# lmcinnes/enstop

Measured on AMD Instinct MI355X. Metric: EM iterations/sec, higher is better.
Workload: dtype f32; 1 GPU; 1M x 100k, 100M nnz; corpus=independent Zipf tokens (SURVEY 8d), nnz=100435863, k=64, schedule=fused, parallelism=single fit

## Files before the change

### enstop_amd/_lib.py

```python
import ctypes as C
import os

import numpy as np

_HERE = os.path.dirname(os.path.abspath(__file__))
LIB_PATH = os.environ.get("ENSTOP_AMD_LIB", os.path.join(_HERE, "libplsa_hip.so"))

PLSA_FUSED = 1
PLSA_TRACE_LL = 4
PLSA_SW_LL_ONLY = 8
PLSA_STOP_NO_ZERO_ARM = 16
PLSA_SHARDED = 64
PLSA_REFERENCE_SUMS = 256
PLSA_REFERENCE_LL = 512

_i32p = np.ctypeslib.ndpointer(np.int32, flags="C_CONTIGUOUS")
_i64p = np.ctypeslib.ndpointer(np.int64, flags="C_CONTIGUOUS")
_f32p = np.ctypeslib.ndpointer(np.float32, flags="C_CONTIGUOUS")
_f64p = np.ctypeslib.ndpointer(np.float64, flags="C_CONTIGUOUS")
_ctx = C.c_void_p
_i64 = C.c_int64
_i32 = C.c_int32
_vp = C.c_void_p

# ... 40 lines not shown
    "plsa_comm_init": (C.c_int, [_ctx, C.c_char_p, _i32, _i32]),
    "plsa_comm_destroy": (C.c_int, [_ctx]),
    "plsa_comm_info": (C.c_int, [_ctx, C.POINTER(_i32), C.POINTER(_i32)]),
    "plsa_comm_barrier": (C.c_int, [_ctx]),
    "plsa_stack_reserve": (C.c_int, [_ctx, C.c_int64, C.c_int64, C.c_int32, C.POINTER(C.c_void_p)]),
    "plsa_comm_allgather_stack": (C.c_int, [_ctx, C.c_int64, C.c_int64, C.c_int32, C.POINTER(C.POINTER(C.c_float))]),
    "plsa_comm_allgather_stack_to": (C.c_int, [_ctx, _i64, _i64, _i32, _f32p]),
    "plsa_comm_allgather_host": (C.c_int, [_ctx, _vp, _i64, _vp]),
    "plsa_comm_allreduce_f64": (C.c_int, [_ctx, _f64p, _i64, _i32]),
    "plsa_comm_broadcast_host": (C.c_int, [_ctx, _vp, _i64, _i32]),
    "plsa_allreduce_accumulator": (C.c_int, [_ctx]),
    "plsa_reference_chain_info": (C.c_int, [_ctx, C.POINTER(_i64), C.POINTER(_i64), C.POINTER(_i32)]),
    "plsa_placement_info": (C.c_int, [_ctx, C.POINTER(_i32), C.POINTER(C.c_double), C.POINTER(C.c_double)]),
    "plsa_schedule_info": (C.c_int, [_ctx, C.POINTER(_i32), C.POINTER(C.c_double), C.POINTER(_i32), C.POINTER(_i32),
                                     C.POINTER(C.c_int64)]),
    "plsa_release_scratch": (C.c_int, [_ctx]),
    "plsa_timing_enable": (C.c_int, [_ctx, _i32]),
    "plsa_timing_reset": (C.c_int, [_ctx]),
    "plsa_timing_get": (C.c_int, [_ctx, C.c_char_p, C.POINTER(C.c_double), C.POINTER(_i64)]),
    "plsa_timing_report": (C.c_int, [_ctx, C.c_char_p, _i64]),
    "plsa_measure_stream_bandwidth": (C.c_int, [_ctx, _i64, _i32, _i32, C.POINTER(C.c_double)]),
    "plsa_all_pairs_hellinger": (C.c_int, [_ctx, C.c_void_p, _i64, _i64, _f64p]),
    "plsa_all_pairs_kl": (C.c_int, [_ctx, C.c_void_p, _i64, _i64, _f64p]),
    "plsa_cluster_representatives": (C.c_int, [_ctx, C.c_void_p, _i64, _i64, _i32p, _vp, _i32, _f32p]),
    "plsa_host_normalize_rows": (None, [_f64p, _i64, _i64]),
    "plsa_host_mt19937_jump": (C.c_int, [C.POINTER(C.c_uint32), _i32]),
    "plsa_generate_synthetic": (C.c_int, [_ctx, _i64, _i64, _i64, C.c_double, C.c_uint64,
                                          C.POINTER(_i64)]),
    "plsa_generate_synthetic_topics": (C.c_int, [_ctx, _i64, _i64, _i64, C.c_double, C.c_uint64, _i32, C.c_double,
                                                 C.c_double, C.POINTER(_i64)]),
# ... 54 lines not shown
```

### enstop_amd/csrc/plsa_hip.hip

```cpp
#include <hip/hip_runtime.h>
#include <hipcub/hipcub.hpp>
#include <rccl/rccl.h>

#include <algorithm>
#include <cmath>
#include <cstdarg>
#include <cstdio>
#include <cstdlib>
#include <cstring>
#include <mutex>
#include <string>
#include <thread>
#include <type_traits>
#include <vector>

#include "../../include/plsa_hip.h"
#include "../../include/plsa_hip_diag.h"
#include "mt_jump.hpp"
#include "plsa_kernels.hpp"
#include "plsa_ref_kernels.hpp"
#include "plsa_synth.hpp"

using plsa::i64;

// ... 30 lines not shown

    i64 bn = 0, bm = 0, bnnz = 0;
    DevBuf b_indptr, b_col, b_val;
    bool active_is_base = true;
    i64 n = 0, m = 0, nnz = 0;
    DevBuf a_indptr, a_col, a_val, rowidx;
    const int *indptr = nullptr, *col = nullptr;
    const float *val = nullptr;
    bool rowidx_valid = false;

    bool csc_valid = false;
    int seg = 256, seg_override = 0, struct_lpn = 0;
    i64 n_items = 0;
    DevBuf colptr, csc_row, csc_val, csc_pos, item_first, item_col, item_start, item_order, partial, heavy_cols;
    bool use_item_order = true, xcd_split = true;
    int chunks_per_lane = 2;
    int row_lpn = 1, row_ch = 1;
    bool row_shape_8x2 = true;
    bool p_borrowed = false;
    bool p_lent = false;
    int e_rows = -1;
    int mt_streams = 256;
    i64 mt_min_blocks = 4096;
    int heavy_items = 32, n_heavy = 0;

    bool force_wide = false;
    bool ritems_valid = false, use_ritems = false;
    int rseg = 64, rseg_override = 0, ritems_mode = -1;
    i64 n_ritems = 0;
    DevBuf ritem_first, ritem_row, ritem_start, rpartial;
// ... 384 lines not shown
int grid_for(plsa_ctx *c, i64 work_items, int items_per_block) {
    i64 need = (work_items + items_per_block - 1) / items_per_block;
    if (need < 1) need = 1;
    return (int)std::min<i64>(need, c->grid_cap);
}

void set_active_pointers(plsa_ctx *c) {
    if (c->active_is_base) {
        c->indptr = c->b_indptr.as<int>(); c->col = c->b_col.as<int>(); c->val = c->b_val.as<float>();
        c->n = c->bn; c->m = c->bm; c->nnz = c->bnnz;
    } else {
        c->indptr = c->a_indptr.as<int>(); c->col = c->a_col.as<int>(); c->val = c->a_val.as<float>();
    }
    c->rowidx_valid = false;
    c->csc_valid = false;
    c->roworder_valid = false;
    c->ritems_valid = false;
    c->eitems_valid = false;
    c->p_valid = false;
    c->ref_pairs_off = false;
    c->ref_heavy_valid = false;
    c->ref_tsum_valid = false;
}

int ensure_rowidx(plsa_ctx *c) {
    if (c->rowidx_valid) return 0;
    CHK(ensure(c, c->rowidx, sizeof(int) * (size_t)c->nnz));
    if (c->n > 0) {
        Scope s(c, "k_expand_rows");
        hipLaunchKernelGGL(plsa::k_expand_rows, dim3(grid_for(c, c->n, 4)), dim3(256), 0, c->stream,
// ... 116 lines not shown
    {
        const i64 slots = (i64)c->prop.multiProcessorCount * 32 * (64 / std::max(1, c->lpn));
        i64 want = c->nnz / std::max<i64>(slots + slots / 4, 1);
        int seg = 16;
        const int cap = 64;
        while (seg * 2 <= want && seg < cap) seg *= 2;
        c->seg = c->seg_override ? c->seg_override : seg;
    }
    const i64 nnz = c->nnz, m = c->m;
    CHK(ensure(c, c->colptr, sizeof(int) * (size_t)(m + 1)));
    CHK(ensure(c, c->csc_row, sizeof(int) * (size_t)nnz));
    CHK(ensure(c, c->csc_val, sizeof(float) * (size_t)nnz));
    CHK(ensure(c, c->csc_pos, sizeof(int) * (size_t)nnz));
    CHK(ensure(c, c->tmp0, sizeof(int) * (size_t)std::max<i64>(nnz, m + 1)));
    CHK(ensure(c, c->tmp1, sizeof(int) * (size_t)nnz));
    if (nnz > 0) {
        hipLaunchKernelGGL(plsa::k_iota, dim3(grid_for(c, nnz, 256)), dim3(256), 0, c->stream,
                           c->tmp1.as<int>(), nnz);
        int bits = 1;
        while (((i64)1 << bits) < m) ++bits;
        size_t bytes = 0;
        HIPCHK(c, hipcub::DeviceRadixSort::SortPairs(nullptr, bytes, c->col, c->tmp0.as<int>(),
                                                     c->tmp1.as<int>(), c->csc_pos.as<int>(), nnz, 0,
                                                     bits, c->stream));
        CHK(ensure(c, c->cubtmp, bytes));
        HIPCHK(c, hipcub::DeviceRadixSort::SortPairs(c->cubtmp.p, bytes, c->col, c->tmp0.as<int>(),
                                                     c->tmp1.as<int>(), c->csc_pos.as<int>(), nnz, 0,
                                                     bits, c->stream));
        hipLaunchKernelGGL(plsa::k_colptr_from_sorted, dim3((unsigned)((m + 256) / 256)), dim3(256), 0, c->stream,
                           c->tmp0.as<int>(), nnz, (int)m, c->colptr.as<int>());
        hipLaunchKernelGGL(plsa::k_csc_gather, dim3(grid_for(c, nnz, 256)), dim3(256), 0, c->stream,
                           c->csc_pos.as<int>(), c->rowidx.as<int>(), c->val, nnz,
                           c->csc_row.as<int>(), c->csc_val.as<float>());
        CHK(launch_check(c, "k_csc_gather"));
    } else {
        HIPCHK(c, hipMemsetAsync(c->colptr.p, 0, sizeof(int) * (size_t)(m + 1), c->stream));
    }
    CHK(ensure(c, c->item_first, sizeof(int) * (size_t)(m + 1)));
    HIPCHK(c, hipMemsetAsync(c->tmp0.p, 0, sizeof(int) * (size_t)(m + 1), c->stream));
    hipLaunchKernelGGL(plsa::k_col_item_counts, dim3((unsigned)((m + 255) / 256)), dim3(256), 0, c->stream,
                       c->colptr.as<int>(), (int)m, c->seg, c->tmp0.as<int>());
    CHK(exclusive_sum_int(c, c->tmp0.as<int>(), c->item_first.as<int>(), m + 1));
    int n_items = 0;
    HIPCHK(c, hipMemcpyAsync(&n_items, c->item_first.as<int>() + m, sizeof(int), hipMemcpyDeviceToHost,
                             c->stream));
    HIPCHK(c, hipStreamSynchronize(c->stream));
    c->n_items = n_items;
    const size_t ni = (size_t)std::max<i64>(n_items, 1);
// ... 27 lines not shown
    CHK(ensure(c, c->item_rec, sizeof(int4) * ni));
    if (n_items > 0) {
        hipLaunchKernelGGL(plsa::k_item_records, dim3((unsigned)((n_items + 255) / 256)), dim3(256), 0, c->stream,
                           c->use_item_order ? c->item_order.as<int>() : nullptr, c->item_col.as<int>(),
                           c->item_start.as<int>(), c->item_end.as<int>(), (i64)n_items, c->item_rec.as<int4>());
        CHK(launch_check(c, "k_item_records"));
    }
    c->bal_valid = false;
    CHK(ensure(c, c->heavy_cols, sizeof(int) * (size_t)(m + 1)));
    HIPCHK(c, hipMemsetAsync(c->heavy_cols.as<int>() + m, 0, sizeof(int), c->stream));
    hipLaunchKernelGGL(plsa::k_heavy_list, dim3((unsigned)((m + 255) / 256)), dim3(256), 0, c->stream,
                       c->item_first.as<int>(), (int)m, c->heavy_items, c->heavy_cols.as<int>(),
                       c->heavy_cols.as<int>() + m);
    CHK(launch_check(c, "k_heavy_list"));
    HIPCHK(c, hipMemcpyAsync(&c->n_heavy, c->heavy_cols.as<int>() + m, sizeof(int), hipMemcpyDeviceToHost, c->stream));
    HIPCHK(c, hipStreamSynchronize(c->stream));
    c->csc_valid = true;
    return 0;
}

int upload_sw(plsa_ctx *c, const float *sw, const float **d_sw) {
    *d_sw = nullptr;
    if (!sw) {
        if (c->sw_resident) {
            if (c->sw_n != c->n) return fail(c, "resident sample weights were set for %lld documents, the active matrix has %lld",
                                              (long long)c->sw_n, (long long)c->n);
            *d_sw = c->sw_res.as<float>();
        }
        return 0;
    }
    CHK(ensure(c, c->sw, sizeof(float) * (size_t)c->n));
    HIPCHK(c, hipMemcpyAsync(c->sw.p, sw, sizeof(float) * (size_t)c->n, hipMemcpyHostToDevice, c->stream));
// ... 109 lines not shown
    CHK(ensure_ritems(c));
    const bool items = c->use_ritems && c->n_ritems > 0;
    int grid = grid_for(c, items ? c->n_ritems : c->n, 256 / c->row_lpn);
    const int *order = nullptr;
    const int gpb_row = 256 / c->row_lpn;
    const bool xcd_rows = !items && !from_p && c->sort_rows && row_xcd_range(c) > 0;
    if (xcd_rows) grid = (int)(((c->n + gpb_row - 1) / gpb_row + 7) / 8 * 8);
    if (!items) CHK(ensure_roworder(c, &order));
    if (items) CHK(ensure(c, c->rpartial, sizeof(float) * (size_t)c->n_ritems * c->kp));
    const int *ri_row = items ? c->ritem_row.as<int>() : nullptr;
    const int *ri_start = items ? c->ritem_start.as<int>() : nullptr;
    float *rpart = items ? c->rpartial.as<float>() : nullptr;
    const int rseg = c->rseg;
    const i64 n_ritems = c->n_ritems;
    if (want_ll) CHK(ensure(c, c->ll_partials, sizeof(double) * (size_t)grid));
    CHK(dispatch_shape_row(c, [&](auto S) {
        using Sh = decltype(S);
        const int *ip = c->indptr, *cl = c->col;
        const float *vl = c->val, *U = c->U[c->cu].as<float>(), *Vt = c->Vt[c->cv].as<float>();
        const float *P = p_base(c);
        float *Un = c->U[out_u(c)].as<float>();
        double *llp = c->ll_partials.as<double>();
        const int n = (int)c->n, kp = c->kp;
        auto go = [&](auto FP, auto LL, auto TN, const char *name) {
            Scope s(c, name);
            hipLaunchKernelGGL((plsa::k_row_pass<Sh, decltype(FP)::value, decltype(LL)::value, decltype(TN)::value>),
                               dim3(grid), dim3(256), 0, c->ls, ip, cl, vl, n, order, U, Vt, P, Un,
                               d_sw, d_norm_pdz, kp, thresh, llp, ri_row, ri_start, rseg, n_ritems, rpart, xcd_rows ? 1 : 0);
        };
        using T = std::true_type;
        using F = std::false_type;
        const bool tiny = thresh < plsa::TINY_THRESH;
        if (from_p) go(T{}, F{}, F{}, "k_row_pass<P>");
        else if (want_ll) { if (tiny) go(F{}, T{}, T{}, "k_row_pass<fused,LL>"); else go(F{}, T{}, F{}, "k_row_pass<fused,LL>"); }
        else { if (tiny) go(F{}, F{}, T{}, "k_row_pass<fused>"); else go(F{}, F{}, F{}, "k_row_pass<fused>"); }
        if (items) {
            Scope s(c, "k_row_reduce");
            hipLaunchKernelGGL((plsa::k_row_reduce<Sh>), dim3(grid_for(c, c->n, 256 / Sh::LPN)), dim3(256), 0, c->ls,
                               c->ritem_first.as<int>(), n, rpart, Un, d_norm_pdz, kp);
        }
    }));
    CHK(launch_check(c, "k_row_pass"));
    if (ll_blocks) *ll_blocks = grid;
// ... 76 lines not shown
                tot += size[x];
            }
            double acc = 0.0;
            for (int x = 0; x < 8; ++x) { acc += size[x]; c->bal_frac[x + 1] = acc / tot; }
            c->bal_frac[8] = 1.0;
            balance_set_lo(c, n_chunks);
            HIPCHK(c, hipMemcpyAsync(c->xcd_lo.p, c->bal_lo, sizeof(int) * 9, hipMemcpyHostToDevice, c->ls));
        }
        c->bal_have_frac = true;
    }
    c->bal_valid = true;
    return 0;
}

int run_col_pass(plsa_ctx *c, bool from_p, const float *d_sw, float thresh, int parts = 3) {
    CHK(ensure_csc(c));
    CHK(ensure(c, c->partial, sizeof(float) * (size_t)std::max<i64>(c->n_items, 1) * c->kp));
    int rc = 0;
    CHK(dispatch_shape_gather(c, table_is_wide(c, c->n), [&](auto S) {
        using Sh = decltype(S);
        constexpr int LPN = Sh::LPN, GPB = 256 / LPN;
        const i64 n_visit = c->n_items;
        const int n_chunks = (int)((n_visit + GPB - 1) / GPB);
        const int grid2 = grid_for(c, c->m, GPB);
        const bool u_fits_l2 = (double)c->n * c->kp * 4.0 <= 2.0 * 1024 * 1024;
        const int xcd_split = (c->xcd_split && n_chunks >= 64 && !u_fits_l2) ? 1 : 0;
        if (parts & 1) {
            rc = ensure(c, c->colsum_rows, sizeof(double) * (size_t)std::max(n_chunks, 1) * c->kp);
            if (rc) return;
            const size_t smem = sizeof(double) * (size_t)GPB * c->kp;
            auto launch = [&](bool timed) -> int {
                int grid = col_grid(c, n_chunks, xcd_split != 0);
                if (c->small_grid > 0 && (double)c->nnz * c->kp < c->overlap_full_limit)
                    grid = std::min(grid, c->small_grid * c->prop.multiProcessorCount);
                Scope s(c, from_p ? "k_col_pass<P>" : "k_col_pass<fused>");
                const int4 *rec = c->item_rec.as<int4>();
                const int *lo = c->xcd_lo.as<int>(), *cr = c->csc_row.as<int>(), *cp = c->csc_pos.as<int>();
                const float *cvl = c->csc_val.as<float>(), *U = c->U[c->cu].as<float>(), *Vt = c->Vt[c->cv].as<float>();
                float *part = c->partial.as<float>();
                double *sums = c->colsum_rows.as<double>();
                unsigned long long *te = c->t_end.as<unsigned long long>();
                const int kp = c->kp;
                auto go = [&](auto FP, auto TM, auto TN) {
                    hipLaunchKernelGGL((plsa::k_col_pass<Sh, decltype(FP)::value, decltype(TM)::value, decltype(TN)::value>),
                                       dim3(grid), dim3(256), smem, c->ls, rec, n_visit, lo, cr, cvl, cp, U, Vt, p_base(c), d_sw,
                                       part, kp, thresh, xcd_split, sums, te);
                };
                using T = std::true_type;
                using F = std::false_type;
                const bool tiny = !from_p && thresh < plsa::TINY_THRESH;
                if (from_p) { if (timed) go(T{}, T{}, F{}); else go(T{}, F{}, F{}); }
                else if (tiny) { if (timed) go(F{}, T{}, T{}); else go(F{}, F{}, T{}); }
                else { if (timed) go(F{}, T{}, F{}); else go(F{}, F{}, F{}); }
                return launch_check(c, "k_col_pass");
            };
            rc = ensure_balance(c, n_chunks, xcd_split != 0, launch);
            if (rc) return;
            rc = launch(false);
            if (rc) return;
            c->colsum_rows_used = n_chunks;
        }
// ... 498 lines not shown
        (tail_prio ? hipStreamCreateWithPriority(&c->stream2, hipStreamNonBlocking, prio_hi)
                   : hipStreamCreateWithFlags(&c->stream2, hipStreamNonBlocking)) != hipSuccess ||
        hipEventCreateWithFlags(&c->ev_fork, hipEventDisableTiming) != hipSuccess ||
        hipEventCreateWithFlags(&c->ev_join, hipEventDisableTiming) != hipSuccess ||
        hipEventCreateWithFlags(&c->ev_row, hipEventDisableTiming) != hipSuccess ||
        hipEventCreateWithFlags(&c->ev_tail, hipEventDisableTiming) != hipSuccess ||
        hipEventCreateWithFlags(&c->ev_ll, hipEventDisableTiming) != hipSuccess ||
        hipHostMalloc((void **)&c->h_ll, sizeof(double) * 2, hipHostMallocDefault) != hipSuccess) {
        delete c;
        return fail(nullptr, "stream / pinned buffer creation failed");
    }
    c->ls = c->stream;
    if (const char *s = getenv("PLSA_OVERLAP")) c->overlap = atoi(s) != 0;
    if (const char *s = getenv("PLSA_OVERLAP_FULL_LIMIT")) c->overlap_full_limit = atof(s);
    if (const char *s = getenv("PLSA_ROW_ITEMS")) c->ritems_mode = atoi(s);
    if (const char *s = getenv("PLSA_ROW_SEG")) c->rseg_override = std::max(1, atoi(s));
    int mult = 128;
    if (const char *s = getenv("PLSA_GRID_MULT")) mult = std::max(1, atoi(s));
    c->grid_cap = c->prop.multiProcessorCount * mult;
    if (const char *s = getenv("PLSA_CONTIG")) g_contig = atoi(s) != 0;
    if (const char *s = getenv("PLSA_PLACEMENT_CANDIDATES")) c->placement_candidates = std::max(1, atoi(s));
    if (const char *s = getenv("PLSA_COL_SEG")) c->seg_override = std::max(1, atoi(s));
    if (const char *s = getenv("PLSA_HEAVY_ITEMS")) c->heavy_items = std::max(1, atoi(s));
    if (const char *s = getenv("PLSA_SORT_ROWS")) c->sort_rows = atoi(s) != 0;
    if (const char *s = getenv("PLSA_ROW_XCD")) c->row_xcd = atoi(s) != 0;
    if (const char *s = getenv("PLSA_ITEM_ORDER")) c->use_item_order = atoi(s) != 0;
    if (const char *s = getenv("PLSA_XCD_SPLIT")) c->xcd_split = atoi(s) != 0;
    if (const char *s = getenv("PLSA_BALANCE")) c->balance = atoi(s);
    if (const char *s = getenv("PLSA_ORDER_BAND")) c->order_band = atoi(s);
    if (const char *s = getenv("PLSA_GRAPH")) c->graph = atoi(s) != 0;
// ... 518 lines not shown
        int first_slot = 0;
        auto collect_first = [&]() -> int {
            if (!first_wait) return 0;
            first_wait = false;
            CHK(wait_ll(c, &ll));
            prev = (float)ll;
            if (ll_trace) ll_trace[first_slot] = prev;
            return 0;
        };
        auto advance = [&]() {
            if (c->rot3) { c->cu = (c->cu + 1) % 3; c->cv = (c->cv + 1) % 3; } else { c->cu ^= 1; c->cv ^= 1; }
        };
        auto enqueue_iteration = [&](bool want_ll, int *blocks) -> int {
            const bool overlap = c->overlap && !c->sharded;
            if (overlap && (double)c->nnz * c->kp < c->overlap_full_limit) {
                CHK(ensure_csc(c));
                CHK(ensure_ritems(c));
                const int *unused = nullptr;
                if (!c->use_ritems) CHK(ensure_roworder(c, &unused));
                if (pipelined) {
                    HIPCHK(c, hipStreamWaitEvent(c->stream, c->ev_tail, 0));
                    HIPCHK(c, hipStreamWaitEvent(c->stream2, c->ev_row, 0));
                    c->ls = c->stream2;
                    int rc = run_col_pass(c, false, d_sw_m, thresh, 1);
                    if (!rc) rc = run_col_tail(c);
                    c->ls = c->stream;
                    if (rc) return rc;
                    HIPCHK(c, hipEventRecord(c->ev_tail, c->stream2));
                    CHK(run_row_pass(c, false, want_ll, d_sw, thresh, nullptr, blocks));
                    HIPCHK(c, hipEventRecord(c->ev_row, c->stream));
                    return 0;
// ... 467 lines not shown
    if (best_gbps) *best_gbps = c->placement_gbps[0];
    if (worst_gbps) *worst_gbps = c->placement_gbps[1];
    return 0;
}

int plsa_schedule_info(plsa_ctx *c, int32_t *xcd_lo, double *xcd_end_us, int32_t *timed_launches, int32_t *item_len,
                       int64_t *n_items) {
    if (xcd_lo) for (int x = 0; x <= 8; ++x) xcd_lo[x] = c->bal_valid ? c->bal_lo[x] : 0;
    if (xcd_end_us) for (int x = 0; x < 8; ++x) xcd_end_us[x] = c->bal_launches > 0 ? c->bal_end_us[x] : 0.0;
    if (timed_launches) *timed_launches = c->bal_launches;
    if (item_len) *item_len = c->csc_valid ? c->seg : 0;
    if (n_items) *n_items = c->csc_valid ? c->n_items : 0;
    return 0;
}

int plsa_release_scratch(plsa_ctx *c) {
    HIPCHK(c, hipSetDevice(c->device));
    HIPCHK(c, hipStreamSynchronize(c->stream));
    if (!c->p_borrowed) release(c->P);
    c->p_lent = false;
    release(c->ref_terms); release(c->ref_csum); release(c->ref_pairs); release(c->ref_exps); release(c->ref_ll_neg); release(c->ref_heavy); release(c->ref_pairs2); release(c->ref_exps2); release(c->ref_tsum);
    release(c->partial); release(c->tmp0); release(c->tmp1); release(c->tmp2); release(c->cubtmp);
    release(c->mt_words); release(c->mt_state); release(c->mt_fin); release(c->mt_poly); release(c->mt_seq);
    release(c->comm_stack); release(c->comm_recv); release(c->comm_send);
    c->p_valid = false;
    c->p_shift = 0;
    return 0;
}

int plsa_timing_enable(plsa_ctx *c, int32_t on) {
    if (!on) CHK(timing_flush(c));
    c->timing = on != 0;
    return 0;
}

int plsa_timing_reset(plsa_ctx *c) {
    CHK(timing_flush(c));
// ... 342 lines not shown
```

### enstop_amd/csrc/plsa_kernels.hpp

```cpp
#pragma once
#include <hip/hip_runtime.h>
#include <stdint.h>

#ifndef PLSA_UNR
#define PLSA_UNR 4
#endif
#ifndef PLSA_NT_STREAMS
#define PLSA_NT_STREAMS 0
#endif
#ifndef PLSA_UNR_E
#define PLSA_UNR_E 16
#endif
#ifndef PLSA_WAVES
#define PLSA_WAVES 1
#endif
#ifndef PLSA_UNR_COL
#define PLSA_UNR_COL 8
#endif
#ifndef PLSA_WAVES_COL
#define PLSA_WAVES_COL PLSA_WAVES
#endif

namespace plsa {

// ... 33 lines not shown
__device__ __forceinline__ int ldi(const int *p) { return PLSA_NT_STREAMS ? __builtin_nontemporal_load(p) : *p; }
__device__ __forceinline__ float ldf(const float *p) { return PLSA_NT_STREAMS ? __builtin_nontemporal_load(p) : *p; }

template <int LPN_, int CH_, bool FULL_, bool WIDE_ = false>
struct Shape {
    static constexpr int LPN = LPN_, CH = CH_;
    static constexpr bool FULL = FULL_, WIDE = WIDE_;
    static constexpr int UNR = (LPN_ <= 8 && CH_ == 1) ? LPN_ : ((LPN_ < PLSA_UNR) ? LPN_ : PLSA_UNR);
    static constexpr int UNR_COL = (LPN_ < PLSA_UNR_COL) ? LPN_ : PLSA_UNR_COL;
    static constexpr int UNR_EF = (LPN_ < 4) ? LPN_ : 4;
    static constexpr int UNR_E_CAP = (PLSA_UNR_E / CH_ > 0) ? PLSA_UNR_E / CH_ : 1;
    static constexpr int UNR_E = (LPN_ < UNR_E_CAP) ? LPN_ : UNR_E_CAP;
    __device__ static __forceinline__ int kp(int kp_rt) { return FULL_ ? 4 * LPN_ * CH_ : kp_rt; }
    __device__ static __forceinline__ int c4(int li, int j) { return 4 * (li + LPN_ * j); }
    __device__ static __forceinline__ bool ok(int li, int j, int kp) { return FULL_ || c4(li, j) < kp; }
};

template <class S, bool ZERO_INVALID, bool STREAM = false>
__device__ __forceinline__ void load_row(const float *row, int li, int kp, float4 (&out)[S::CH]) {
#pragma unroll
    for (int j = 0; j < S::CH; ++j) {
        const bool ok = S::ok(li, j, kp);
        const float *p = row + (ok ? S::c4(li, j) : 0);
        const float4 v = STREAM ? ld4_nt(p) : ld4(p);
        out[j] = (ZERO_INVALID && !ok) ? zero4() : v;
    }
}

template <class S>
__device__ __forceinline__ void gather_row(const float *table, int row, int li, int kp, float4 (&out)[S::CH]) {
    if constexpr (S::WIDE) {
// ... 181 lines not shown
    double ll = 0.0;
    const i64 first_block = xcd_rows ? (i64)(blockIdx.x & 7) * (gridDim.x >> 3) + (blockIdx.x >> 3) : (i64)blockIdx.x;
    constexpr bool tiny = !FROM_P && TINY;
    const bool items = ritem_row != nullptr;
    const i64 n_work = items ? n_ritems : (i64)n;
    for (i64 r = first_block * GPB + gid; r < n_work; r += (i64)gridDim.x * GPB) {
        const int d = items ? ritem_row[r] : (row_order ? row_order[r] : (int)r);
        const int j0 = items ? ritem_start[r] : indptr[d];
        const int j1 = items ? min(j0 + rseg, indptr[d + 1]) : indptr[d + 1];
        float4 u[CH], acc[CH];
        load_row<S, true, PLSA_NT_STREAMS>(U + (i64)d * kp, li, kp, u);
#pragma unroll
        for (int j = 0; j < CH; ++j) acc[j] = zero4();
        const float swd = (WANT_LL && sw) ? sw[d] : 1.0f;
        int w_n = (j0 + li < j1) ? ldi(colidx + j0 + li) : 0;
        float x_n = (j0 + li < j1) ? ldf(vals + j0 + li) : 0.f;
        for (int jb = j0; jb < j1; jb += LPN) {
            const int w_l = w_n;
            const float x_l = x_n;
            const int jn = jb + LPN + li;
            w_n = jn < j1 ? ldi(colidx + jn) : 0;
            x_n = jn < j1 ? ldf(vals + jn) : 0.f;
            const int cnt = min(LPN, j1 - jb);
            for (int s0 = 0; s0 < cnt; s0 += UNR) {
                float4 a[UNR][CH];
                float x[UNR];
                constexpr bool OWNER = !FROM_P && UNR == LPN;
#pragma unroll
                for (int q = 0; q < UNR; ++q) {
                    const int w = __shfl(w_l, s0 + q, LPN);
                    if (!OWNER) x[q] = __shfl(x_l, s0 + q, LPN);
                    if (FROM_P) load_row<S, false>(P + (i64)min(jb + s0 + q, j1 - 1) * kp, li, kp, a[q]);
                    else gather_row<S>(Vt, w, li, kp, a[q]);
                }
                float my_dot = 1.f, my_x = 0.f;
                if (OWNER) {
                    float nmine = 0.f;
// ... 233 lines not shown
    const int nq = xcd_split ? (int)((gridDim.x + 7 - xcd) / 8) : (int)gridDim.x;
    const int q = xcd_split ? (int)(blockIdx.x >> 3) : (int)blockIdx.x;
    const int c_lo = xcd_split ? xcd_lo[xcd] : 0, c_hi = xcd_split ? xcd_lo[xcd + 1] : n_chunks;
    if (TIMED && blockIdx.x == 0 && threadIdx.x == 0) t_end[gridDim.x] = wall_clock64();
    for (int chunk = c_lo + q; chunk < c_hi; chunk += nq) {
        const i64 io = (i64)chunk * GPB + gid;
        float4 acc[CH];
#pragma unroll
        for (int j = 0; j < CH; ++j) acc[j] = zero4();
        if (io < n_items) {
            const int4 rec = item_rec[io];
            const int w = rec.x, j0 = rec.y, j1 = rec.z;
            float4 vt[CH];
            load_row<S, true, PLSA_NT_STREAMS>(Vt + (i64)w * kp, li, kp, vt);
            int d_n = (j0 + li < j1) ? ldi(csc_row + j0 + li) : 0;
            float x_n = (j0 + li < j1) ? ldf(csc_val + j0 + li) : 0.f;
            int p_n = (FROM_P && j0 + li < j1) ? ldi(csc_pos + j0 + li) : 0;
            for (int jb = j0; jb < j1; jb += LPN) {
                const int d_l = d_n, p_l = p_n;
                float x_l = x_n;
                const int jn = jb + LPN + li;
                d_n = jn < j1 ? ldi(csc_row + jn) : 0;
                x_n = jn < j1 ? ldf(csc_val + jn) : 0.f;
                if (FROM_P) p_n = jn < j1 ? ldi(csc_pos + jn) : 0;
                if (sw) x_l *= sw[d_l];
                const int cnt = min(LPN, j1 - jb);
                int s0 = 0;
                for (; s0 + UNR <= cnt; s0 += UNR)
                    col_batch<S, FROM_P, UNR, TINY>(s0, d_l, x_l, p_l, li, kp, thresh, U, P, vt, acc);
                constexpr int TAIL = (UNR >= 2 && LPN >= 2) ? 2 : 1;
                for (; s0 < cnt; s0 += TAIL)
                    col_batch<S, FROM_P, TAIL, TINY>(s0, d_l, x_l, p_l, li, kp, thresh, U, P, vt, acc);
            }
#pragma unroll
            for (int j = 0; j < CH; ++j)
                if (S::ok(li, j, kp)) st4(partial + (i64)rec.w * kp + S::c4(li, j), acc[j]);
        }
        block_colsum<S>(acc, li, gid, kp, scol, chunk_sums + (i64)chunk * kp);
// ... 439 lines not shown
        for (int z = lane; z < kp; z += 64) {
            float v = 0.f;
            if (z < k) {
                unsigned long long x = seed ^ ((unsigned long long)r * 0x9E3779B97F4A7C15ull + (unsigned long long)z);
                x += 0x9E3779B97F4A7C15ull; x = (x ^ (x >> 30)) * 0xBF58476D1CE4E5B9ull;
                x = (x ^ (x >> 27)) * 0x94D049BB133111EBull; x ^= x >> 31;
                v = ((float)(x >> 40) + 0.5f) * (1.0f / 16777216.0f);
            }
            A[r * kp + z] = v;
            part += v;
        }
        for (int o = 32; o > 0; o >>= 1) part += __shfl_xor(part, o, 64);
        for (int z = lane; z < k; z += 64) A[r * kp + z] /= part;
    }
}
__global__ void k_csc_gather(const int *__restrict__ pos, const int *__restrict__ rowidx,
                             const float *__restrict__ vals, i64 nnz, int *__restrict__ csc_row,
                             float *__restrict__ csc_val) {
    for (i64 i = (i64)blockIdx.x * blockDim.x + threadIdx.x; i < nnz; i += (i64)gridDim.x * blockDim.x) {
        const int p = pos[i];
        csc_row[i] = rowidx[p];
        csc_val[i] = vals[p];
    }
}
__global__ void k_item_counts(const int *__restrict__ colptr, int m, int seg, int *__restrict__ cnt) {
    const i64 c = (i64)blockIdx.x * blockDim.x + threadIdx.x;
    if (c < m) cnt[c] = (colptr[c + 1] - colptr[c] + seg - 1) / seg;
}
__global__ void k_col_item_counts(const int *__restrict__ colptr, int m, int seg, int *__restrict__ cnt) {
    const i64 c = (i64)blockIdx.x * blockDim.x + threadIdx.x;
    if (c < m) cnt[c] = (colptr[c + 1] - colptr[c] + seg - 1) / seg;
}

__global__ void k_item_fill(const int *__restrict__ colptr, const int *__restrict__ item_first, int m, int seg,
                            const int *__restrict__ csc_row, int *__restrict__ item_col,
                            int *__restrict__ item_start, int *__restrict__ item_end, int band, int len_bits,
                            unsigned long long *__restrict__ item_key, int *__restrict__ item_id, int n_items) {
    const i64 i = (i64)blockIdx.x * blockDim.x + threadIdx.x;
// ... 557 lines not shown
```

### enstop_amd/engine.py

```python
import ctypes as C
import os
import threading

import numpy as np

from . import _lib
from ._lib import (PLSA_FUSED, PLSA_REFERENCE_LL, PLSA_REFERENCE_SUMS, PLSA_SHARDED, PLSA_STOP_NO_ZERO_ARM, PLSA_SW_LL_ONLY,
                   PLSA_TRACE_LL, ptr)


class DeviceError(RuntimeError):
    pass


def default_device():
    if "ENSTOP_AMD_DEVICE" in os.environ:
        return int(os.environ["ENSTOP_AMD_DEVICE"])
    dev = int(os.environ.get("LOCAL_RANK", "0"))
    if dev > 0:
        cnt = C.c_int(0)
        if _lib.load().plsa_device_count(C.byref(cnt)) == 0 and 0 < cnt.value <= dev:
            if cnt.value != 1:
                raise RuntimeError("LOCAL_RANK=%d but only %d GPUs are visible: start one rank per visible GPU, "
                                   "narrow the devices to one per rank (HIP_VISIBLE_DEVICES), or set "
# ... 353 lines not shown
        self._ok(self._L.plsa_reference_chain_info(self._h, C.byref(a), C.byref(b), C.byref(c_)))
        return dict(slow_chunks=a.value, chunks=b.value, serial_chain_now=bool(c_.value))

    def placement_info(self):
        n, a, b = C.c_int32(0), C.c_double(0.0), C.c_double(0.0)
        self._ok(self._L.plsa_placement_info(self._h, C.byref(n), C.byref(a), C.byref(b)))
        return dict(candidates=n.value, kept_fill_GBps=round(a.value, 1), worst_fill_GBps=round(b.value, 1))

    def balance_info(self):
        lo = (C.c_int32 * 9)(); t = (C.c_double * 8)()
        n, seg, items = C.c_int32(0), C.c_int32(0), C.c_int64(0)
        self._ok(self._L.plsa_schedule_info(self._h, lo, t, C.byref(n), C.byref(seg), C.byref(items)))
        return dict(xcd_chunk_boundaries=list(lo), xcd_finish_us=[round(v, 1) for v in t], timed_launches=n.value,
                    item_entries=seg.value, n_items=items.value)

    def release_scratch(self):
        self._ok(self._L.plsa_release_scratch(self._h))

    def timing(self, on=True):
        self._ok(self._L.plsa_timing_enable(self._h, int(on)))

    def timing_reset(self):
        self._ok(self._L.plsa_timing_reset(self._h))

    def timing_get(self, prefix):
        ms, n = C.c_double(0.0), C.c_int64(0)
        self._ok(self._L.plsa_timing_get(self._h, prefix.encode(), C.byref(ms), C.byref(n)))
        return ms.value, n.value

    def stream_bandwidth(self, nbytes=1 << 32, kind=0, reps=5):
# ... 52 lines not shown
```

### include/plsa_hip_diag.h

```cpp
#ifndef PLSA_HIP_DIAG_H
#define PLSA_HIP_DIAG_H

#include "plsa_hip.h"

#ifdef __cplusplus
extern "C" {
#endif

int plsa_hw_queues(void);
int plsa_device_info(plsa_ctx *ctx, char *name64, char *arch64, int *cus, int64_t *hbm_bytes);

int plsa_download_active_csr(plsa_ctx *ctx, int32_t *indptr, int32_t *indices, float *data);

int plsa_init_factors_device(plsa_ctx *ctx, int32_t k, uint64_t seed);

int plsa_mt_marginals(plsa_ctx *ctx, double *out, int32_t k);

int plsa_set_p(plsa_ctx *ctx, const float *P);

int plsa_accumulator_get(plsa_ctx *ctx, float *host);
int plsa_accumulator_set(plsa_ctx *ctx, const float *host);

int plsa_comm_last_error(plsa_ctx *ctx, char *buf, int64_t cap);

int plsa_comm_barrier(plsa_ctx *ctx);
int plsa_comm_allreduce_f64(plsa_ctx *ctx, double *inout, int64_t count, int32_t op);

int plsa_reference_chain_info(plsa_ctx *ctx, int64_t *slow_chunks, int64_t *chunks, int32_t *serial_now);

int plsa_placement_info(plsa_ctx *ctx, int32_t *candidates, double *best_gbps, double *worst_gbps);

int plsa_schedule_info(plsa_ctx *ctx, int32_t *xcd_lo , double *xcd_end_us , int32_t *timed_launches,
                       int32_t *item_len, int64_t *n_items);

int plsa_timing_enable(plsa_ctx *ctx, int32_t on);
int plsa_timing_reset(plsa_ctx *ctx);
int plsa_timing_get(plsa_ctx *ctx, const char *prefix, double *total_ms, int64_t *launches);
int plsa_timing_report(plsa_ctx *ctx, char *buf, int64_t cap);
int plsa_measure_stream_bandwidth(plsa_ctx *ctx, int64_t bytes, int32_t kind, int32_t reps, double *gbps);

void plsa_host_normalize_rows(double *a, int64_t rows, int64_t cols);

int plsa_host_mt19937_jump(uint32_t *key , int32_t log2_blocks);

int plsa_generate_synthetic(plsa_ctx *ctx, int64_t n, int64_t m, int64_t nnz_target, double zipf_s,
                            uint64_t seed, int64_t *nnz_out);
int plsa_generate_synthetic_topics(plsa_ctx *ctx, int64_t n, int64_t m, int64_t nnz_target, double zipf_s,
                                   uint64_t seed, int32_t k0, double alpha, double background, int64_t *nnz_out);
int plsa_synthetic_dominant_topics(plsa_ctx *ctx, int32_t *out );
// ... 6 lines not shown
```

Measured before the change: 318.2 iter/s.

## Pack sparse index and small integer count into one 32-bit word

Builds packed CSR and CSC entry arrays. Each entry holds a 24-bit row or column id in the low bits and an 8-bit integer count in the high bits, with an escape to the float value array when the count is not an integer between 1 and 255. The fused row and column passes read these packed words instead of separate index and value arrays, which cuts sparse-stream traffic from 8 to about 4 bytes per nonzero. Packing is used only when ids fit in 24 bits and escapes are at most 1/16 of entries. It costs extra memory, a one-time packing pass with a host sync, and a branch per entry in the hot loop.

After: 348.5 iter/s, median of 6. +9.5%, better.

```diff
diff --git a/enstop_amd/_lib.py b/enstop_amd/_lib.py
--- a/enstop_amd/_lib.py
+++ b/enstop_amd/_lib.py
@@ -78,6 +78,7 @@
     "plsa_placement_info": (C.c_int, [_ctx, C.POINTER(_i32), C.POINTER(C.c_double), C.POINTER(C.c_double)]),
     "plsa_schedule_info": (C.c_int, [_ctx, C.POINTER(_i32), C.POINTER(C.c_double), C.POINTER(_i32), C.POINTER(_i32),
                                      C.POINTER(C.c_int64)]),
+    "plsa_packed_info": (C.c_int, [_ctx, C.POINTER(_i32), C.POINTER(_i32)]),
     "plsa_release_scratch": (C.c_int, [_ctx]),
     "plsa_timing_enable": (C.c_int, [_ctx, _i32]),
     "plsa_timing_reset": (C.c_int, [_ctx]),
diff --git a/enstop_amd/csrc/plsa_hip.hip b/enstop_amd/csrc/plsa_hip.hip
--- a/enstop_amd/csrc/plsa_hip.hip
+++ b/enstop_amd/csrc/plsa_hip.hip
@@ -68,6 +68,9 @@
     i64 n_items = 0;
     DevBuf colptr, csc_row, csc_val, csc_pos, item_first, item_col, item_start, item_order, partial, heavy_cols;
     bool use_item_order = true, xcd_split = true;
+    bool packed = true;
+    bool pk_csr_valid = false, pk_csr_ok = false, pk_csc_valid = false, pk_csc_ok = false;
+    DevBuf pk_csr, pk_csc, pk_count;
     int chunks_per_lane = 2;
     int row_lpn = 1, row_ch = 1;
     bool row_shape_8x2 = true;
@@ -482,6 +485,8 @@
     }
     c->rowidx_valid = false;
     c->csc_valid = false;
+    c->pk_csr_valid = false;
+    c->pk_csc_valid = false;
     c->roworder_valid = false;
     c->ritems_valid = false;
     c->eitems_valid = false;
@@ -628,6 +633,14 @@
     CHK(ensure(c, c->csc_pos, sizeof(int) * (size_t)nnz));
     CHK(ensure(c, c->tmp0, sizeof(int) * (size_t)std::max<i64>(nnz, m + 1)));
     CHK(ensure(c, c->tmp1, sizeof(int) * (size_t)nnz));
+    const bool pack = c->packed && nnz > 0 && c->n <= plsa::PACK_MAX_IDS;
+    c->pk_csc_valid = false;
+    c->pk_csc_ok = false;
+    if (pack) {
+        CHK(ensure(c, c->pk_csc, sizeof(unsigned) * (size_t)nnz));
+        CHK(ensure(c, c->pk_count, sizeof(unsigned long long)));
+        HIPCHK(c, hipMemsetAsync(c->pk_count.p, 0, sizeof(unsigned long long), c->stream));
+    }
     if (nnz > 0) {
         hipLaunchKernelGGL(plsa::k_iota, dim3(grid_for(c, nnz, 256)), dim3(256), 0, c->stream,
                            c->tmp1.as<int>(), nnz);
@@ -645,7 +658,8 @@
                            c->tmp0.as<int>(), nnz, (int)m, c->colptr.as<int>());
         hipLaunchKernelGGL(plsa::k_csc_gather, dim3(grid_for(c, nnz, 256)), dim3(256), 0, c->stream,
                            c->csc_pos.as<int>(), c->rowidx.as<int>(), c->val, nnz,
-                           c->csc_row.as<int>(), c->csc_val.as<float>());
+                           c->csc_row.as<int>(), c->csc_val.as<float>(), pack ? c->pk_csc.as<unsigned>() : nullptr,
+                           pack ? c->pk_count.as<unsigned long long>() : nullptr);
         CHK(launch_check(c, "k_csc_gather"));
     } else {
         HIPCHK(c, hipMemsetAsync(c->colptr.p, 0, sizeof(int) * (size_t)(m + 1), c->stream));
@@ -703,8 +717,46 @@
                        c->heavy_cols.as<int>() + m);
     CHK(launch_check(c, "k_heavy_list"));
     HIPCHK(c, hipMemcpyAsync(&c->n_heavy, c->heavy_cols.as<int>() + m, sizeof(int), hipMemcpyDeviceToHost, c->stream));
+    unsigned long long escaped = 0;
+    if (pack) HIPCHK(c, hipMemcpyAsync(&escaped, c->pk_count.p, sizeof escaped, hipMemcpyDeviceToHost, c->stream));
     HIPCHK(c, hipStreamSynchronize(c->stream));
     c->csc_valid = true;
+    c->pk_csc_valid = c->packed;
+    c->pk_csc_ok = pack && escaped * 16 <= (unsigned long long)nnz;
+    if (!c->pk_csc_ok) release(c->pk_csc);
+    return 0;
+}
+
+int build_packed(plsa_ctx *c, DevBuf &out, const int *ids, const float *vals, i64 id_range, bool *ok) {
+    *ok = false;
+    const i64 nnz = c->nnz;
+    if (nnz <= 0 || id_range > plsa::PACK_MAX_IDS) { release(out); return 0; }
+    CHK(ensure(c, out, sizeof(unsigned) * (size_t)nnz));
+    CHK(ensure(c, c->pk_count, sizeof(unsigned long long)));
+    HIPCHK(c, hipMemsetAsync(c->pk_count.p, 0, sizeof(unsigned long long), c->stream));
+    hipLaunchKernelGGL(plsa::k_pack_entries, dim3(grid_for(c, nnz, 256)), dim3(256), 0, c->stream,
+                       ids, vals, nnz, out.as<unsigned>(), c->pk_count.as<unsigned long long>());
+    CHK(launch_check(c, "k_pack_entries"));
+    unsigned long long escaped = 0;
+    HIPCHK(c, hipMemcpyAsync(&escaped, c->pk_count.p, sizeof escaped, hipMemcpyDeviceToHost, c->stream));
+    HIPCHK(c, hipStreamSynchronize(c->stream));
+    *ok = escaped * 16 <= (unsigned long long)nnz;
+    if (!*ok) release(out);
+    return 0;
+}
+
+int ensure_packed_csr(plsa_ctx *c) {
+    if (!c->packed || c->pk_csr_valid) return 0;
+    CHK(build_packed(c, c->pk_csr, c->col, c->val, c->m, &c->pk_csr_ok));
+    c->pk_csr_valid = true;
+    return 0;
+}
+
+int ensure_packed_csc(plsa_ctx *c) {
+    CHK(ensure_csc(c));
+    if (!c->packed || c->pk_csc_valid) return 0;
+    CHK(build_packed(c, c->pk_csc, c->csc_row.as<int>(), c->csc_val.as<float>(), c->n, &c->pk_csc_ok));
+    c->pk_csc_valid = true;
     return 0;
 }
 
@@ -844,19 +896,27 @@
     const int rseg = c->rseg;
     const i64 n_ritems = c->n_ritems;
     if (want_ll) CHK(ensure(c, c->ll_partials, sizeof(double) * (size_t)grid));
+    if (!from_p) CHK(ensure_packed_csr(c));
+    const bool packed = !from_p && c->packed && c->pk_csr_ok;
     CHK(dispatch_shape_row(c, [&](auto S) {
         using Sh = decltype(S);
-        const int *ip = c->indptr, *cl = c->col;
+        const int *ip = c->indptr, *cl = packed ? c->pk_csr.as<int>() : c->col;
         const float *vl = c->val, *U = c->U[c->cu].as<float>(), *Vt = c->Vt[c->cv].as<float>();
         const float *P = p_base(c);
         float *Un = c->U[out_u(c)].as<float>();
         double *llp = c->ll_partials.as<double>();
         const int n = (int)c->n, kp = c->kp;
-        auto go = [&](auto FP, auto LL, auto TN, const char *name) {
+        auto launch = [&](auto SS, auto FP, auto LL, auto TN, const char *name) {
             Scope s(c, name);
-            hipLaunchKernelGGL((plsa::k_row_pass<Sh, decltype(FP)::value, decltype(LL)::value, decltype(TN)::value>),
+            hipLaunchKernelGGL((plsa::k_row_pass<decltype(SS), decltype(FP)::value, decltype(LL)::value, decltype(TN)::value>),
                                dim3(grid), dim3(256), 0, c->ls, ip, cl, vl, n, order, U, Vt, P, Un,
                                d_sw, d_norm_pdz, kp, thresh, llp, ri_row, ri_start, rseg, n_ritems, rpart, xcd_rows ? 1 : 0);
+        };
+        auto go = [&](auto FP, auto LL, auto TN, const char *name) {
+            if constexpr (!decltype(FP)::value) {
+                if (packed) { launch(plsa::Packed<Sh>{}, FP, LL, TN, name); return; }
+            }
+            launch(Sh{}, FP, LL, TN, name);
         };
         using T = std::true_type;
         using F = std::false_type;
@@ -963,7 +1023,8 @@
 }
 
 int run_col_pass(plsa_ctx *c, bool from_p, const float *d_sw, float thresh, int parts = 3) {
-    CHK(ensure_csc(c));
+    CHK(from_p ? ensure_csc(c) : ensure_packed_csc(c));
+    const bool packed = !from_p && c->packed && c->pk_csc_ok;
     CHK(ensure(c, c->partial, sizeof(float) * (size_t)std::max<i64>(c->n_items, 1) * c->kp));
     int rc = 0;
     CHK(dispatch_shape_gather(c, table_is_wide(c, c->n), [&](auto S) {
@@ -984,16 +1045,23 @@
                     grid = std::min(grid, c->small_grid * c->prop.multiProcessorCount);
                 Scope s(c, from_p ? "k_col_pass<P>" : "k_col_pass<fused>");
                 const int4 *rec = c->item_rec.as<int4>();
-                const int *lo = c->xcd_lo.as<int>(), *cr = c->csc_row.as<int>(), *cp = c->csc_pos.as<int>();
+                const int *lo = c->xcd_lo.as<int>(), *cp = c->csc_pos.as<int>();
+                const int *cr = packed ? c->pk_csc.as<int>() : c->csc_row.as<int>();
                 const float *cvl = c->csc_val.as<float>(), *U = c->U[c->cu].as<float>(), *Vt = c->Vt[c->cv].as<float>();
                 float *part = c->partial.as<float>();
                 double *sums = c->colsum_rows.as<double>();
                 unsigned long long *te = c->t_end.as<unsigned long long>();
                 const int kp = c->kp;
-                auto go = [&](auto FP, auto TM, auto TN) {
-                    hipLaunchKernelGGL((plsa::k_col_pass<Sh, decltype(FP)::value, decltype(TM)::value, decltype(TN)::value>),
+                auto run = [&](auto SS, auto FP, auto TM, auto TN) {
+                    hipLaunchKernelGGL((plsa::k_col_pass<decltype(SS), decltype(FP)::value, decltype(TM)::value, decltype(TN)::value>),
                                        dim3(grid), dim3(256), smem, c->ls, rec, n_visit, lo, cr, cvl, cp, U, Vt, p_base(c), d_sw,
                                        part, kp, thresh, xcd_split, sums, te);
+                };
+                auto go = [&](auto FP, auto TM, auto TN) {
+                    if constexpr (!decltype(FP)::value) {
+                        if (packed) { run(plsa::Packed<Sh>{}, FP, TM, TN); return; }
+                    }
+                    run(Sh{}, FP, TM, TN);
                 };
                 using T = std::true_type;
                 using F = std::false_type;
@@ -1522,6 +1590,7 @@
     if (const char *s = getenv("PLSA_OVERLAP")) c->overlap = atoi(s) != 0;
     if (const char *s = getenv("PLSA_OVERLAP_FULL_LIMIT")) c->overlap_full_limit = atof(s);
     if (const char *s = getenv("PLSA_ROW_ITEMS")) c->ritems_mode = atoi(s);
+    if (const char *s = getenv("PLSA_PACKED")) c->packed = atoi(s) != 0;
     if (const char *s = getenv("PLSA_ROW_SEG")) c->rseg_override = std::max(1, atoi(s));
     int mult = 128;
     if (const char *s = getenv("PLSA_GRID_MULT")) mult = std::max(1, atoi(s));
@@ -2070,7 +2139,8 @@
         auto enqueue_iteration = [&](bool want_ll, int *blocks) -> int {
             const bool overlap = c->overlap && !c->sharded;
             if (overlap && (double)c->nnz * c->kp < c->overlap_full_limit) {
-                CHK(ensure_csc(c));
+                CHK(ensure_packed_csc(c));
+                CHK(ensure_packed_csr(c));
                 CHK(ensure_ritems(c));
                 const int *unused = nullptr;
                 if (!c->use_ritems) CHK(ensure_roworder(c, &unused));
@@ -2568,6 +2638,12 @@
     return 0;
 }
 
+int plsa_packed_info(plsa_ctx *c, int32_t *csr, int32_t *csc) {
+    if (csr) *csr = !c->packed ? 0 : (c->pk_csr_valid ? (c->pk_csr_ok ? 1 : 0) : -1);
+    if (csc) *csc = !c->packed ? 0 : (c->csc_valid && c->pk_csc_valid ? (c->pk_csc_ok ? 1 : 0) : -1);
+    return 0;
+}
+
 int plsa_release_scratch(plsa_ctx *c) {
     HIPCHK(c, hipSetDevice(c->device));
     HIPCHK(c, hipStreamSynchronize(c->stream));
@@ -2575,6 +2651,9 @@
     c->p_lent = false;
     release(c->ref_terms); release(c->ref_csum); release(c->ref_pairs); release(c->ref_exps); release(c->ref_ll_neg); release(c->ref_heavy); release(c->ref_pairs2); release(c->ref_exps2); release(c->ref_tsum);
     release(c->partial); release(c->tmp0); release(c->tmp1); release(c->tmp2); release(c->cubtmp);
+    release(c->pk_csr); release(c->pk_csc); release(c->pk_count);
+    c->pk_csr_valid = c->pk_csc_valid = false;
+    c->pk_csr_ok = c->pk_csc_ok = false;
     release(c->mt_words); release(c->mt_state); release(c->mt_fin); release(c->mt_poly); release(c->mt_seq);
     release(c->comm_stack); release(c->comm_recv); release(c->comm_send);
     c->p_valid = false;
diff --git a/enstop_amd/csrc/plsa_kernels.hpp b/enstop_amd/csrc/plsa_kernels.hpp
--- a/enstop_amd/csrc/plsa_kernels.hpp
+++ b/enstop_amd/csrc/plsa_kernels.hpp
@@ -71,7 +71,23 @@
     __device__ static __forceinline__ int kp(int kp_rt) { return FULL_ ? 4 * LPN_ * CH_ : kp_rt; }
     __device__ static __forceinline__ int c4(int li, int j) { return 4 * (li + LPN_ * j); }
     __device__ static __forceinline__ bool ok(int li, int j, int kp) { return FULL_ || c4(li, j) < kp; }
+    static constexpr bool PACKED = false;
 };
+
+template <class S>
+struct Packed : S {
+    static constexpr bool PACKED = true;
+};
+constexpr long long PACK_MAX_IDS = 1ll << 24;
+__device__ __forceinline__ unsigned pack_code(float v) {
+    return (v >= 1.f && v <= 255.f && v == truncf(v)) ? (unsigned)v : 0u;
+}
+__device__ __forceinline__ void unpack_entry(int &id, float &x, const float *__restrict__ vals, int j, int j_end) {
+    const unsigned e = (unsigned)id;
+    id = (int)(e & 0xFFFFFFu);
+    x = (float)(e >> 24);
+    if (x == 0.f && j < j_end) x = ldf(vals + j);
+}
 
 template <class S, bool ZERO_INVALID, bool STREAM = false>
 __device__ __forceinline__ void load_row(const float *row, int li, int kp, float4 (&out)[S::CH]) {
@@ -283,13 +299,14 @@
         for (int j = 0; j < CH; ++j) acc[j] = zero4();
         const float swd = (WANT_LL && sw) ? sw[d] : 1.0f;
         int w_n = (j0 + li < j1) ? ldi(colidx + j0 + li) : 0;
-        float x_n = (j0 + li < j1) ? ldf(vals + j0 + li) : 0.f;
+        float x_n = (!S::PACKED && j0 + li < j1) ? ldf(vals + j0 + li) : 0.f;
         for (int jb = j0; jb < j1; jb += LPN) {
-            const int w_l = w_n;
-            const float x_l = x_n;
+            int w_l = w_n;
+            float x_l = x_n;
+            if (S::PACKED) unpack_entry(w_l, x_l, vals, jb + li, j1);
             const int jn = jb + LPN + li;
             w_n = jn < j1 ? ldi(colidx + jn) : 0;
-            x_n = jn < j1 ? ldf(vals + jn) : 0.f;
+            if (!S::PACKED) x_n = jn < j1 ? ldf(vals + jn) : 0.f;
             const int cnt = min(LPN, j1 - jb);
             for (int s0 = 0; s0 < cnt; s0 += UNR) {
                 float4 a[UNR][CH];
@@ -553,14 +570,16 @@
             float4 vt[CH];
             load_row<S, true, PLSA_NT_STREAMS>(Vt + (i64)w * kp, li, kp, vt);
             int d_n = (j0 + li < j1) ? ldi(csc_row + j0 + li) : 0;
-            float x_n = (j0 + li < j1) ? ldf(csc_val + j0 + li) : 0.f;
+            float x_n = (!S::PACKED && j0 + li < j1) ? ldf(csc_val + j0 + li) : 0.f;
             int p_n = (FROM_P && j0 + li < j1) ? ldi(csc_pos + j0 + li) : 0;
             for (int jb = j0; jb < j1; jb += LPN) {
-                const int d_l = d_n, p_l = p_n;
+                int d_l = d_n;
+                const int p_l = p_n;
                 float x_l = x_n;
+                if (S::PACKED) unpack_entry(d_l, x_l, csc_val, jb + li, j1);
                 const int jn = jb + LPN + li;
                 d_n = jn < j1 ? ldi(csc_row + jn) : 0;
-                x_n = jn < j1 ? ldf(csc_val + jn) : 0.f;
+                if (!S::PACKED) x_n = jn < j1 ? ldf(csc_val + jn) : 0.f;
                 if (FROM_P) p_n = jn < j1 ? ldi(csc_pos + jn) : 0;
                 if (sw) x_l *= sw[d_l];
                 const int cnt = min(LPN, j1 - jb);
@@ -1030,14 +1049,38 @@
         for (int z = lane; z < k; z += 64) A[r * kp + z] /= part;
     }
 }
-__global__ void k_csc_gather(const int *__restrict__ pos, const int *__restrict__ rowidx,
-                             const float *__restrict__ vals, i64 nnz, int *__restrict__ csc_row,
-                             float *__restrict__ csc_val) {
+__device__ __forceinline__ void add_escapes(unsigned esc, unsigned long long *__restrict__ n_esc) {
+    for (int o = 32; o > 0; o >>= 1) esc += __shfl_xor(esc, o, 64);
+    if ((threadIdx.x & 63) == 0 && esc) atomicAdd(n_esc, (unsigned long long)esc);
+}
+__global__ __launch_bounds__(256) void k_pack_entries(const int *__restrict__ ids, const float *__restrict__ vals, i64 nnz,
+                                                      unsigned *__restrict__ packed, unsigned long long *__restrict__ n_esc) {
+    unsigned esc = 0;
+    for (i64 i = (i64)blockIdx.x * blockDim.x + threadIdx.x; i < nnz; i += (i64)gridDim.x * blockDim.x) {
+        const unsigned code = pack_code(vals[i]);
+        packed[i] = (unsigned)ids[i] | (code << 24);
+        esc += code == 0u;
+    }
+    add_escapes(esc, n_esc);
+}
+__global__ __launch_bounds__(256) void k_csc_gather(const int *__restrict__ pos, const int *__restrict__ rowidx,
+                                                    const float *__restrict__ vals, i64 nnz, int *__restrict__ csc_row,
+                                                    float *__restrict__ csc_val, unsigned *__restrict__ packed,
+                                                    unsigned long long *__restrict__ n_esc) {
+    unsigned esc = 0;
     for (i64 i = (i64)blockIdx.x * blockDim.x + threadIdx.x; i < nnz; i += (i64)gridDim.x * blockDim.x) {
         const int p = pos[i];
-        csc_row[i] = rowidx[p];
-        csc_val[i] = vals[p];
-    }
+        const int r = rowidx[p];
+        const float v = vals[p];
+        csc_row[i] = r;
+        csc_val[i] = v;
+        if (packed) {
+            const unsigned code = pack_code(v);
+            packed[i] = (unsigned)r | (code << 24);
+            esc += code == 0u;
+        }
+    }
+    if (packed) add_escapes(esc, n_esc);
 }
 __global__ void k_item_counts(const int *__restrict__ colptr, int m, int seg, int *__restrict__ cnt) {
     const i64 c = (i64)blockIdx.x * blockDim.x + threadIdx.x;
diff --git a/enstop_amd/engine.py b/enstop_amd/engine.py
--- a/enstop_amd/engine.py
+++ b/enstop_amd/engine.py
@@ -391,6 +391,12 @@
         return dict(xcd_chunk_boundaries=list(lo), xcd_finish_us=[round(v, 1) for v in t], timed_launches=n.value,
                     item_entries=seg.value, n_items=items.value)
 
+    def packed_info(self):
+        a, b = C.c_int32(0), C.c_int32(0)
+        self._ok(self._L.plsa_packed_info(self._h, C.byref(a), C.byref(b)))
+        name = {1: "packed", 0: "arrays", -1: None}
+        return dict(csr=name[a.value], csc=name[b.value])
+
     def release_scratch(self):
         self._ok(self._L.plsa_release_scratch(self._h))
 
diff --git a/include/plsa_hip_diag.h b/include/plsa_hip_diag.h
--- a/include/plsa_hip_diag.h
+++ b/include/plsa_hip_diag.h
@@ -33,6 +33,8 @@
 int plsa_schedule_info(plsa_ctx *ctx, int32_t *xcd_lo , double *xcd_end_us , int32_t *timed_launches,
                        int32_t *item_len, int64_t *n_items);
 
+int plsa_packed_info(plsa_ctx *ctx, int32_t *csr, int32_t *csc);
+
 int plsa_timing_enable(plsa_ctx *ctx, int32_t on);
 int plsa_timing_reset(plsa_ctx *ctx);
 int plsa_timing_get(plsa_ctx *ctx, const char *prefix, double *total_ms, int64_t *launches);
```
